# eovs/ldpc-lib

Hardware: AMD Instinct MI355X
Metric: decoded frames/sec, (2048,1024) QC-LDPC, 50 iters min-sum (higher is better)
Workload: dtype f64

## Files before the change

### include/ldpc_hip.h

```cpp
#ifndef LDPC_HIP_H
#define LDPC_HIP_H

#include <stdint.h>

#ifdef __cplusplus
extern "C" {
#endif

#define LDPC_HIP_ABI_VERSION 4

#define LDPC_HIP_BP_DEC 0
#define LDPC_HIP_SP_DEC 1
#define LDPC_HIP_ASP_DEC 2
#define LDPC_HIP_MS_DEC 3
#define LDPC_HIP_IMS_DEC 4
#define LDPC_HIP_IASP_DEC 5
#define LDPC_HIP_FHT_DEC 6
#define LDPC_HIP_TASP_DEC 7
#define LDPC_HIP_LMS_DEC 8
#define LDPC_HIP_LCHE_DEC 9

#define LDPC_HIP_EINVAL (-1)
#define LDPC_HIP_EUNSUPPORTED (-2)
#define LDPC_HIP_EHIP (-3)
// ... 4 lines not shown
int ldpc_hip_abi_version(void);
const char *ldpc_hip_last_error(void);
int ldpc_hip_device_count(void);

int ldpc_hip_open(int decoder_id, int rh, int nh, int M, const int16_t *hd, int device, ldpc_hip_ctx **out);
void ldpc_hip_close(ldpc_hip_ctx *ctx);

int ldpc_hip_n(const ldpc_hip_ctx *ctx);
int ldpc_hip_r(const ldpc_hip_ctx *ctx);
int ldpc_hip_edges(const ldpc_hip_ctx *ctx);
int ldpc_hip_hard_words(const ldpc_hip_ctx *ctx);
const char *ldpc_hip_kernel_name(const ldpc_hip_ctx *ctx);
int ldpc_hip_set_jit_mode(int mode);
int ldpc_hip_set_jit_mode_thread(int mode);
const char *ldpc_hip_last_launch(const ldpc_hip_ctx *ctx);

int ldpc_hip_decode_dev(ldpc_hip_ctx *ctx, const double *d_llr, long long B, int maxiter, double alpha,
                        uint32_t *d_hard, int32_t *d_iters, double *d_soft, void *stream);

int ldpc_hip_set_bp_chain(ldpc_hip_ctx *ctx, int on, int reset_carry);

int ldpc_hip_set_ims_params(ldpc_hip_ctx *ctx, double thr, int qbits, int dbits);

int ldpc_hip_decode_host(ldpc_hip_ctx *ctx, double *llr, long long B, int maxiter, int decision, double alpha,
                         double *decword, int32_t *iters, int clobber_sp_input);


int ldpc_hip_set_interleaver(ldpc_hip_ctx *ctx, int permutation_type, int permutation_block, int permutation_inter);
int ldpc_hip_set_codewords(ldpc_hip_ctx *ctx, const uint8_t *codewords, int ncw);

// ... 163 lines not shown
```

### ldpc-lib_amd/csrc/aot/ms_m64.hip

```cpp
#include "../ldpc_aot.hpp"

LDPC_AOT_KERNEL(ms_spec_appendix_c_m64_kernel, ms_m64_body, CodeAppendixCM64, 64, 2)
```

### ldpc-lib_amd/csrc/ldpc_aot.hpp

```cpp
#pragma once

#include <hip/hip_runtime.h>

#include "ldpc_spec.hpp"
#include "code_appendix_c_m64.hpp"

#define LDPC_AOT_DECLARE(name, threads, waves_per_simd) \
    __global__ void __launch_bounds__(threads, waves_per_simd) name(const ldpc_spec::SpecArgs a);
#define LDPC_AOT_KERNEL(name, body, Code, threads, waves_per_simd)                                   \
    __global__ void __launch_bounds__(threads, waves_per_simd) name(const ldpc_spec::SpecArgs a) {   \
        ldpc_spec::body<ldpc_spec::Code>(a);                                                         \
    }

LDPC_AOT_DECLARE(ms_spec_appendix_c_m64_kernel, 64, 2)
LDPC_AOT_DECLARE(ms_spec_appendix_c_m126_kernel, 128, 2)
LDPC_AOT_DECLARE(ms_chunk_appendix_c_m126_kernel, 64, 1)
LDPC_AOT_DECLARE(ms_spec_appendix_c_m512_kernel, 512, 2)
LDPC_AOT_DECLARE(ims_spec_appendix_c_m64_kernel, 64, 3)
LDPC_AOT_DECLARE(ims_spec_appendix_c_m126_kernel, 128, 2)
LDPC_AOT_DECLARE(lms_spec_appendix_c_m64_kernel, 64, 2)
LDPC_AOT_DECLARE(lms_spec_appendix_c_m512_kernel, 512, 2)
LDPC_AOT_DECLARE(sp_spec_appendix_c_m64_kernel, 512, 4)
LDPC_AOT_DECLARE(bp_spec_appendix_c_m64_kernel, 512, 4)
LDPC_AOT_DECLARE(asp_spec_appendix_c_m64_kernel, 512, 4)
LDPC_AOT_DECLARE(iasp_spec_appendix_c_m64_kernel, 512, 4)
LDPC_AOT_DECLARE(tasp_spec_appendix_c_m64_kernel, 128, 2)
LDPC_AOT_DECLARE(lche_spec_appendix_c_m64_kernel, 128, 2)
LDPC_AOT_DECLARE(tasp_spec_appendix_c_m126_kernel, 256, 2)
```

### ldpc-lib_amd/csrc/ldpc_hip.hip

```cpp
#include "../../include/ldpc_hip.h"
#include "../../include/ldpc/interleaver.h"
#include "../../include/ldpc/encoder.h"

#include <hip/hip_runtime.h>

#include <algorithm>
#include <cmath>
#include <cstdarg>
#include <cstdio>
#include <cstdlib>
#include <cstring>
#include <atomic>
#include <memory>
#include <string>
#include <type_traits>
#include <vector>

#include "ldpc_frontend.hpp"
#include "ldpc_jit.hpp"
#include "ldpc_kernels.hpp"
#include "ldpc_codeset.hpp"
#include "ldpc_codeset_wide.hpp"
#include "ldpc_codeset_sp.hpp"
#include "ldpc_global.hpp"
// ... 87 lines not shown
        for (int j = 0; same && j < rh; ++j) {
            same = (row_start[j + 1] - row_start[j]) == FC::RW[j];
            for (int e = row_start[j]; same && e < row_start[j + 1]; ++e)
                same = (int)(edges[e] >> 16) == FC::COL[j][e - row_start[j]] && (int)(edges[e] & 0xffffu) == FC::SH[j][e - row_start[j]];
        }
        return same;
    }
};

struct AotInstance {
    int decoder;
    const void *fn;
    int threads;
    const char *name;
    bool (CodeTables::*matches)() const;
};
const AotInstance kAot[] = {
    {LDPC_HIP_MS_DEC, (const void *)ms_spec_appendix_c_m64_kernel, 64, "ms_spec_appendix_c_m64_kernel", &CodeTables::is<ldpc_spec::CodeAppendixCM64>},
    {LDPC_HIP_MS_DEC, (const void *)ms_spec_appendix_c_m126_kernel, 128, "ms_spec_appendix_c_m126_kernel", &CodeTables::is<ldpc_spec::CodeAppendixCM126>},
    {LDPC_HIP_MS_DEC, (const void *)ms_chunk_appendix_c_m126_kernel, 64, "ms_chunk_appendix_c_m126_kernel", &CodeTables::is<ldpc_spec::CodeAppendixCM126>},
    {LDPC_HIP_MS_DEC, (const void *)ms_spec_appendix_c_m512_kernel, 512, "ms_spec_appendix_c_m512_kernel", &CodeTables::is<ldpc_spec::CodeAppendixCM512>},
    {LDPC_HIP_IMS_DEC, (const void *)ims_spec_appendix_c_m64_kernel, 64, "ims_spec_appendix_c_m64_kernel", &CodeTables::is<ldpc_spec::CodeAppendixCM64>},
    {LDPC_HIP_IMS_DEC, (const void *)ims_spec_appendix_c_m126_kernel, 128, "ims_spec_appendix_c_m126_kernel", &CodeTables::is<ldpc_spec::CodeAppendixCM126>},
    {LDPC_HIP_LMS_DEC, (const void *)lms_spec_appendix_c_m64_kernel, 64, "lms_spec_appendix_c_m64_kernel", &CodeTables::is<ldpc_spec::CodeAppendixCM64>},
    {LDPC_HIP_LMS_DEC, (const void *)lms_spec_appendix_c_m512_kernel, 512, "lms_spec_appendix_c_m512_kernel", &CodeTables::is<ldpc_spec::CodeAppendixCM512>},
    {LDPC_HIP_SP_DEC, (const void *)sp_spec_appendix_c_m64_kernel, 64 * ldpc_spec::kSpBodyWaves, "sp_spec_appendix_c_m64_kernel", &CodeTables::is<ldpc_spec::CodeAppendixCM64>},
    {LDPC_HIP_BP_DEC, (const void *)bp_spec_appendix_c_m64_kernel, 512, "bp_spec_appendix_c_m64_kernel", &CodeTables::is<ldpc_spec::CodeAppendixCM64>},
    {LDPC_HIP_ASP_DEC, (const void *)asp_spec_appendix_c_m64_kernel, 512, "asp_spec_appendix_c_m64_kernel", &CodeTables::is<ldpc_spec::CodeAppendixCM64>},
    {LDPC_HIP_IASP_DEC, (const void *)iasp_spec_appendix_c_m64_kernel, 512, "iasp_spec_appendix_c_m64_kernel", &CodeTables::is<ldpc_spec::CodeAppendixCM64>},
    {LDPC_HIP_LCHE_DEC, (const void *)lche_spec_appendix_c_m64_kernel, 128, "lche_spec_appendix_c_m64_kernel", &CodeTables::is<ldpc_spec::CodeAppendixCM64>},
    {LDPC_HIP_TASP_DEC, (const void *)tasp_spec_appendix_c_m64_kernel, 128, "tasp_spec_appendix_c_m64_kernel", &CodeTables::is<ldpc_spec::CodeAppendixCM64>},
    {LDPC_HIP_TASP_DEC, (const void *)tasp_spec_appendix_c_m126_kernel, 256, "tasp_spec_appendix_c_m126_kernel", &CodeTables::is<ldpc_spec::CodeAppendixCM126>},
};
// ... 73 lines not shown
    bool multiwave = false;
    bool have_generic = false;
    size_t lds_bytes = 0;
    double ims_thr = 1.4;
    int ims_qbits = 6, ims_dbits = 8;
    bool asp_cw2 = false;
    bool global_tier = false;
    char *d_glob_ws = nullptr;
    size_t glob_stride = 0;
    int glob_grid = 0;
    bool fast_m64 = false;
    int variant = 2;
    ldpc::FastTab fast_tab;
    const void *spec_aot = nullptr;
    const ldpc_jit::Kernel *spec_jit = nullptr;
    int spec_threads = 64;
    int spec_frames_per_block = 1;
    size_t spec_lds = 0;
    std::shared_ptr<ldpc_jit::Job> jit_job;
    std::string jit_name;
    bool global_is_fallback = false;
    unsigned *d_queue = nullptr;
    int persist_grid = 0;
    bool persist_jit = false;
    std::string kernel_name;
    std::string generic_name;
    const char *last_launch = "";
    bool bp_chain = true;
    std::vector<uint32_t> bp_carry;
    uint32_t *d_bp_stale = nullptr, *d_bp_synd = nullptr;
    int32_t *d_bp_idx = nullptr;
    long long bp_frames = 0;
    double *d_ims_coef = nullptr;
    long long ims_coef_frames = 0;
    int32_t *d_row_start = nullptr, *d_col_start = nullptr;
    uint32_t *d_edges = nullptr, *d_col_edges = nullptr, *d_col_slot = nullptr, *d_edge_row = nullptr;
    double *w_llr = nullptr;
    uint32_t *w_hard = nullptr;
    int32_t *w_iters = nullptr;
    double *w_soft = nullptr;
    unsigned long long *w_counters = nullptr;
    long long w_frames = 0;
// ... 95 lines not shown
        HIP_TRY(hipEventRecord(ev0, stream));
        return 0;
    }
    int end() {
        if (!c) return 0;
        HIP_TRY(hipEventRecord(ev1, stream));
        c->events.emplace_back(ev0, ev1);
        ev0 = ev1 = nullptr;
        return 0;
    }
    ~ProfTimer() { for (hipEvent_t e : {ev0, ev1}) if (e) (void)hipEventDestroy(e); }
};

struct SpecPlan { const char *body = nullptr; int threads = 0; size_t lds = 0; bool required = false; int frames_per_block = 1; };

constexpr size_t kLdsBudget = 160 * 1024 - 64;

int tasp_lane_regs(const CodeTables &t) {
    int regs = 85;
    for (int j = 0; j < t.rh; ++j) { const int L = (t.row_start[j + 1] - t.row_start[j] + 1) / 2; regs += 2 * L + (L + 1) / 2; }
    return regs;
}

SpecPlan plan_spec(int decoder_id, const CodeTables &t) {
    SpecPlan p;
    const int M = t.M, N = t.nh * t.M, W = (M + 63) / 64;
    const size_t soft_lds = sizeof(double) * (size_t)N + 16;
    if (!t.all_cols_used || t.max_rw > 16 || t.rh > 64 || t.nh > 64) return p;
    switch (decoder_id) {
    case LDPC_HIP_MS_DEC:
        if (M == 64) { p.body = "ms_m64_body"; p.threads = 64; p.lds = ldpc_spec::kMsM64LdsBytes((size_t)N); }
        else if (M <= 32) {
            p.body = "ms_small_body"; p.threads = 64; p.frames_per_block = 64 / M; p.lds = sizeof(double) * (size_t)N * (size_t)(64 / M);
        }
        else if (M > 64 && M <= 128 && !(getenv("LDPC_HIP_MS_CHUNK") && atoi(getenv("LDPC_HIP_MS_CHUNK")) == 0)) {
            p.body = "ms_chunk_body"; p.threads = 64; p.lds = sizeof(double) * (size_t)N;
        }
        else if (M >= 33 && M <= 512 && soft_lds <= kLdsBudget) { p.body = "ms_body"; p.threads = 64 * W; p.lds = soft_lds; }
        break;
    case LDPC_HIP_LMS_DEC:
        if (M <= 32) {
            p.body = "lms_small_body"; p.threads = 64; p.frames_per_block = 64 / M; p.lds = sizeof(double) * (size_t)N * (size_t)(64 / M);
        } else if (M >= 33 && M <= 512 && soft_lds <= kLdsBudget) { p.body = "lms_body"; p.threads = 64 * W; p.lds = soft_lds; }
        break;
    case LDPC_HIP_IMS_DEC: {
        const size_t lds = (((size_t)2 * N + 15) & ~(size_t)15) + (size_t)t.rh * 2 * LDPC_IMS_MSG_COPIES * M * 4 + 16;
// ... 140 lines not shown
        ga.d.ims_thr = c->ims_thr; ga.d.ims_qbits = c->ims_qbits; ga.d.ims_dbits = c->ims_dbits;
    }
    auto glaunch = [&](long long slots, const ChainIo &io) -> int {
        ga.slots = slots; ga.stale = io.stale; ga.synd_out = io.synd_out; ga.frame_idx = io.frame_idx;
        if (io.iters) ga.d.iters = io.iters;
        hipLaunchKernelGGL(kind.global, dim3((unsigned)(slots < grid ? slots : grid)), dim3((unsigned)ldpc::glob_threads(c->N)), 0, d.stream, ga);
        HIP_TRY(hipGetLastError());
        return 0;
    };
    if (c->decoder_id == LDPC_HIP_BP_DEC && c->bp_chain) return run_bp_chain(c, d.B, d.iters, d.stream, glaunch);
    ChainIo io;
    io.iters = d.iters;
    return glaunch(d.B, io);
}

int launch_spec(ldpc_hip_ctx *c, const decoder_kind &kind, const DecodeCall &d) {
    ldpc_spec::SpecArgs sa{};
    if (c->decoder_id == LDPC_HIP_IMS_DEC) {
        if (int rc = ims_scale(c, d.llr, d.B, d.stream)) return rc;
        sa.ims_coef = c->d_ims_coef; sa.ims_thr = c->ims_thr;
        sa.ims_max_quant = (1 << (c->ims_qbits - 1)) - 1; sa.ims_max_data = (1 << (c->ims_dbits - 1)) - 1; sa.ims_ialpha = ims_ialpha(d.alpha);
    }
    sa.llr = d.llr; sa.hard = d.hard; sa.iters = d.iters; sa.soft_out = d.soft; sa.maxiter = d.maxiter; sa.alpha = d.alpha;
    sa.nframes = d.B;
    static const bool persist_on = !(getenv("LDPC_HIP_PERSISTENT") && atoi(getenv("LDPC_HIP_PERSISTENT")) == 0);
    const bool persistent = persist_on && c->spec_frames_per_block == 1 && kind.queue;
    if (persistent) {
        if (!c->d_queue) HIP_TRY(hipMalloc(&c->d_queue, 64));
        if (c->persist_grid == 0 || c->persist_jit != (c->spec_aot == nullptr)) {
            int per_cu = 0, cus = 0;
            if (c->spec_aot) { if (int rc = set_lds_limit(c->spec_aot, c->spec_lds)) return rc; }
            hipError_t e = c->spec_aot ? hipOccupancyMaxActiveBlocksPerMultiprocessor(&per_cu, c->spec_aot, c->spec_threads, c->spec_lds)
                                       : hipModuleOccupancyMaxActiveBlocksPerMultiprocessor(&per_cu, c->spec_jit->fn, c->spec_threads, c->spec_lds);
            if (e != hipSuccess || per_cu < 1) { (void)hipGetLastError(); per_cu = 1; }
            HIP_TRY(hipDeviceGetAttribute(&cus, hipDeviceAttributeMultiprocessorCount, c->device));
            c->persist_grid = per_cu * (cus > 0 ? cus : 256);
            c->persist_jit = c->spec_aot == nullptr;
        }
    }
    auto launch = [&](long long frames) -> int {
        long long blocks = (frames + c->spec_frames_per_block - 1) / c->spec_frames_per_block;
        if (persistent && blocks > c->persist_grid) {
            HIP_TRY(hipMemsetAsync(c->d_queue, 0, sizeof(unsigned), d.stream));
            sa.queue = c->d_queue;
            blocks = c->persist_grid;
        }
        void *kargs[] = {&sa};
        if (c->spec_aot) {
            if (int rc = set_lds_limit(c->spec_aot, c->spec_lds)) return rc;
            HIP_TRY(hipLaunchKernel(c->spec_aot, dim3((unsigned)blocks), dim3((unsigned)c->spec_threads), kargs, c->spec_lds, d.stream));
        } else {
            HIP_TRY(hipModuleLaunchKernel(c->spec_jit->fn, (unsigned)blocks, 1, 1, (unsigned)c->spec_threads, 1, 1, (unsigned)c->spec_lds,
                                          d.stream, kargs, nullptr));
        }
        return 0;
    };
    if (c->decoder_id == LDPC_HIP_BP_DEC && c->bp_chain)
        return run_bp_chain(c, d.B, d.iters, d.stream, [&](long long frames, const ChainIo &io) -> int {
            sa.stale = io.stale; sa.synd_out = io.synd_out; sa.frame_idx = io.frame_idx; sa.iters = io.iters;
            return launch(frames);
        });
    return launch(d.B);
}

int launch_generic(ldpc_hip_ctx *c, const decoder_kind &kind, const DecodeCall &d) {
    ldpc::DecArgs a{};
    a.llr = d.llr; a.hard = d.hard; a.iters = d.iters; a.soft_out = d.soft;
// ... 87 lines not shown

    c->have_generic = have_generic;
    if (have_generic) c->generic_name = c->kernel_name;

    c->asp_cw2 = t.all_cw2;
    const bool can_global = !kind->global_min_rw2 || t.min_rw >= 2;
    const char *genv = getenv("LDPC_HIP_FORCE_GLOBAL");
    const bool forced_global = genv && atoi(genv) != 0;

    const SpecPlan plan = plan_spec(decoder_id, t);
    std::string why_not = plan.body ? "" : "this code shape has no code-specialised kernel";
    if (plan.body && (c->variant >= 2 || plan.required)) {
        c->spec_threads = plan.threads; c->spec_lds = plan.lds; c->spec_frames_per_block = plan.frames_per_block;
        for (const AotInstance &inst : kAot)
            if (inst.decoder == decoder_id && inst.threads == plan.threads && (t.*inst.matches)()) {
                c->spec_aot = inst.fn;
                c->kernel_name = std::string(inst.name) + " (ahead of time)";
                break;
            }
        const int jit_mode = jit_mode_effective();
        if (!c->spec_aot && jit_mode != 0 && !forced_global) {
            const bool has_fallback = have_generic || can_global;
            if (jit_mode == 2 && has_fallback) {
                c->spec_jit = ldpc_jit::get(device, plan.body, t.rows(), nh, M, why_not, false);
                if (!c->spec_jit) {
                    auto job = std::make_shared<ldpc_jit::Job>();
                    job->device = device; job->nh = nh; job->M = M; job->body = plan.body; job->rows = t.rows();
                    ldpc_jit::Worker::instance().submit(job);
                    c->jit_job = job;
                    c->jit_name = std::string(plan.body) + " instance (hiprtc)";
                    why_not = "its hiprtc instance is being compiled in the background";
                }
            } else {
                c->spec_jit = ldpc_jit::get(device, plan.body, t.rows(), nh, M, why_not);
            }
            if (c->spec_jit) c->kernel_name = std::string(plan.body) + " instance (hiprtc)";
        } else if (!c->spec_aot) {
            why_not = forced_global ? "LDPC_HIP_FORCE_GLOBAL" : "LDPC_HIP_JIT=0";
        }
    }
    if (can_global && (forced_global || (!c->spec_aot && !c->spec_jit && !have_generic))) {
        c->global_tier = true;
        c->global_is_fallback = c->jit_job != nullptr;
        c->spec_aot = nullptr; c->spec_jit = nullptr;
        c->kernel_name = kind->global_name;
    }
    if (c->global_tier || decoder_id == LDPC_HIP_IMS_DEC)
        c->glob_stride = ldpc::glob_ws_bytes(c->N, c->R, t.ne, M, kind->glob_edge_arrays);
    if (!c->spec_aot && !c->spec_jit && !c->global_tier) {
        if (!have_generic)
            return fail(LDPC_HIP_EUNSUPPORTED, "decoder %d, code %dx%d lifting %d: not supported by the generic kernel (limits: %d block rows, "
                        "%d block columns, row weight %d, M <= 512, 160 KiB LDS), no code-specialised instance: %s; the shape-unlimited "
                        "tier serves every built decoder; decoders 2, 5 and 7 need row weights >= 2, decoder 9 row weights <= 1024",
                        decoder_id, rh, nh, M, kRHM, kNHM, kRWM, why_not.c_str());
        if (plan.body && c->variant >= 2 && !c->jit_job)
// ... 9 lines not shown
    };
    HIP_TRY(upload(&c->d_row_start, t.row_start));
    HIP_TRY(upload(&c->d_col_start, t.col_start));
    HIP_TRY(upload(&c->d_edges, t.edges));
    HIP_TRY(upload(&c->d_col_edges, t.col_edges));
    HIP_TRY(upload(&c->d_col_slot, t.col_slot));
    HIP_TRY(upload(&c->d_edge_row, t.edge_row));
    HIP_TRY(hipMalloc(&c->w_counters, sizeof(unsigned long long) * 8));
    *out = c.release();
    return 0;
}

void ldpc_hip_close(ldpc_hip_ctx *c) {
    if (!c) return;
    if (c->jit_job) c->jit_job->cancelled.store(true);
    (void)hipSetDevice(c->device);
    free_workspace(c);
    if (c->d_row_start) (void)hipFree(c->d_row_start);
    if (c->d_col_start) (void)hipFree(c->d_col_start);
    if (c->d_edges) (void)hipFree(c->d_edges);
    if (c->d_col_edges) (void)hipFree(c->d_col_edges);
    if (c->d_col_slot) (void)hipFree(c->d_col_slot);
    if (c->d_edge_row) (void)hipFree(c->d_edge_row);
    if (c->w_counters) (void)hipFree(c->w_counters);
    if (c->d_queue) (void)hipFree(c->d_queue);
    if (c->d_ims_coef) (void)hipFree(c->d_ims_coef);
    if (c->d_bp_stale) (void)hipFree(c->d_bp_stale);
    if (c->d_bp_synd) (void)hipFree(c->d_bp_synd);
    if (c->d_bp_idx) (void)hipFree(c->d_bp_idx);
    if (c->d_glob_ws) (void)hipFree(c->d_glob_ws);
// ... 19 lines not shown
    adopt_jit(const_cast<ldpc_hip_ctx *>(c));
    return c->kernel_name.c_str();
}

int ldpc_hip_set_jit_mode(int mode) {
    if (mode < 0 || mode > 2) return fail(LDPC_HIP_EINVAL, "ldpc_hip_set_jit_mode: 0 (never), 1 (inside ldpc_hip_open) or 2 (in the background)");
    return g_jit_mode.exchange(mode);
}
int ldpc_hip_set_jit_mode_thread(int mode) {
    if (mode < -1 || mode > 2) return fail(LDPC_HIP_EINVAL, "ldpc_hip_set_jit_mode_thread: -1 (no override), 0, 1 or 2");
    const int before = t_jit_mode;
    t_jit_mode = mode;
    return before;
}
const char *ldpc_hip_last_launch(const ldpc_hip_ctx *c) { return c ? c->last_launch : ""; }

int ldpc_hip_decode_dev(ldpc_hip_ctx *c, const double *d_llr, long long B, int maxiter, double alpha,
                        uint32_t *d_hard, int32_t *d_iters, double *d_soft, void *stream_) {
    if (!c || B < 0) return fail(LDPC_HIP_EINVAL, "ldpc_hip_decode_dev: bad argument");
    if (B == 0) return 0;
    if (!d_llr) return fail(LDPC_HIP_EINVAL, "ldpc_hip_decode_dev: null llr");
    if (B > 0x7fffffffLL) return fail(LDPC_HIP_EINVAL, "batch too large");
    if (maxiter < 1) return fail(LDPC_HIP_EINVAL, "ldpc_hip_decode_dev: maxiter must be >= 1 (got %d)", maxiter);
    if (int rc = set_device(c)) return rc;
    hipStream_t stream = (hipStream_t)stream_;
    adopt_jit(c);

    ProfTimer timer;
    if (int rc = timer.begin(c, stream)) return rc;
    const decoder_kind &kind = *decoder_find(c->decoder_id);
    const DecodeCall d{d_llr, B, maxiter, alpha, d_hard, d_iters, d_soft, stream};
    bool use_spec = c->spec_aot || c->spec_jit;
    bool use_global = c->global_tier;
    const int ialpha = ims_ialpha(alpha);
    if (use_spec && c->decoder_id == LDPC_HIP_IMS_DEC && (c->ims_dbits > 8 || c->ims_qbits > 8 || ialpha < 0 || ialpha > 16)) {
        use_spec = false;
        if (!c->have_generic) use_global = true;
    }
    c->last_launch = use_global ? kind.global_name : use_spec ? c->kernel_name.c_str() : c->generic_name.c_str();
    if (int rc = use_global ? launch_global(c, kind, d) : use_spec ? launch_spec(c, kind, d) : launch_generic(c, kind, d)) return rc;
    HIP_TRY(hipGetLastError());
    return timer.end();
}

int ldpc_hip_decode_host(ldpc_hip_ctx *c, double *llr, long long B, int maxiter, int decision, double alpha,
                         double *decword, int32_t *iters, int clobber_sp_input) {
    if (!c || !llr || B < 0) return fail(LDPC_HIP_EINVAL, "ldpc_hip_decode_host: bad argument");
    if (B == 0) return 0;
    if (int rc = set_device(c)) return rc;
    const decoder_kind &kind = *decoder_find(c->decoder_id);
    const bool sp = kind.soft_is_input;
    if (kind.ignores_decision) decision = 0;
    const bool need_soft = decision != 0 || (sp && clobber_sp_input);
    if (int rc = ensure_workspace(c, B, need_soft)) return rc;
// ... 448 lines not shown
```

### ldpc-lib_amd/csrc/ldpc_jit.hpp

```cpp
#pragma once

#include <dlfcn.h>
#include <sys/stat.h>
#include <unistd.h>
#include <hip/hip_runtime.h>

#include <atomic>
#include <condition_variable>
#include <cstdio>
#include <cstdlib>
#include <deque>
#include <fstream>
#include <iterator>
#include <map>
#include <memory>
#include <mutex>
#include <sstream>
#include <string>
#include <thread>
#include <vector>

namespace ldpc_jit {

struct Kernel {
// ... 65 lines not shown
      << "    static constexpr int SH[" << rh << "][" << wmax << "] = {" << sh.str() << "};\n"
      << "    static constexpr int FIRST[" << rh << "][" << wmax << "] = {" << fi.str() << "};\n"
      << "};\n";
    return o.str();
}

inline std::string this_library_dir() {
    Dl_info info;
    if (!dladdr(reinterpret_cast<void *>(&this_library_dir), &info) || !info.dli_fname) return ".";
    std::string p = info.dli_fname;
    const size_t k = p.find_last_of('/');
    return k == std::string::npos ? "." : p.substr(0, k);
}

inline const Kernel *get(int device, const char *body, const std::vector<std::vector<std::pair<int, int>>> &rows, int nh,
                         int M, std::string &err, bool compile = true) {
    static std::mutex mu;
    static std::map<std::string, Kernel> &cache = *new std::map<std::string, Kernel>();
    const std::string code = code_struct(rows, nh, M);
    const bool eight_waves = std::string(body) == "sp_body" || std::string(body) == "asp_body" || std::string(body) == "iasp_body" ||
                             std::string(body) == "bp_body";
    const bool tasp = std::string(body) == "tasp_body" || std::string(body) == "lche_body";
    int tasp_regs = 85;
    for (const auto &r : rows) tasp_regs += 2 * (((int)r.size() + 1) / 2) + (((int)r.size() + 1) / 2 + 1) / 2;
    const int threads = eight_waves ? 512 : std::string(body) == "ms_chunk_body" ? 64 : tasp ? ((2 * M + 63) / 64) * 64 : ((M + 63) / 64) * 64;
    const std::string key = std::to_string(device) + "|" + body + "|" + code;
    auto lookup = [&]() -> const Kernel * {
        std::lock_guard<std::mutex> lk(mu);
        auto it = cache.find(key);
        return it != cache.end() ? &it->second : nullptr;
    };
// ... 13 lines not shown
    const std::string hdr = hs.str();
    const std::string tab_path = this_library_dir() + "/csrc/lche_table.hpp";
    std::ifstream tf(tab_path);
    if (!tf) { err = "cannot read " + tab_path; return nullptr; }
    std::stringstream ts;
    ts << tf.rdbuf();
    const std::string tab = ts.str();
    const std::string src = "#include \"ldpc_spec.hpp\"\nnamespace {\n" + code +
                            "}\nextern \"C\" __global__ void __launch_bounds__(" + std::to_string(threads) + (eight_waves ? ", 4" : ((tasp && tasp_regs > 256) || std::string(body) == "ms_chunk_body") ? ", 1" : ", 2") + ") spec_jit(const ldpc_spec::SpecArgs a) {\n"
                            "    ldpc_spec::" + body + "<Code>(a);\n}\n";
    std::string cache_file;
    std::string cache_dir;
    if (const char *dir = getenv("LDPC_HIP_CACHE_DIR")) cache_dir = dir;
    else if (const char *x = getenv("XDG_CACHE_HOME")) cache_dir = std::string(x) + "/ldpc_hip";
    else if (const char *h = getenv("HOME")) cache_dir = std::string(h) + "/.cache/ldpc_hip";
    if (cache_dir == "off" || cache_dir == "0") cache_dir.clear();
    if (!cache_dir.empty()) {
        for (size_t i = 1; i <= cache_dir.size(); ++i)
            if (i == cache_dir.size() || cache_dir[i] == '/') (void)mkdir(cache_dir.substr(0, i).c_str(), 0755);
        const char *dir = cache_dir.c_str();
        unsigned long long h = 1469598103934665603ull;
        auto mix = [&](const std::string &t) { for (unsigned char ch : t) { h ^= ch; h *= 1099511628211ull; } };
        mix(src); mix(hdr); mix(tab); mix("gfx950 -O3 -ffp-contract=off");
        int rt_version = 0;
        (void)hipRuntimeGetVersion(&rt_version);
        mix("rt" + std::to_string(rt_version));
        hipDeviceProp_t prop;
        if (hipGetDeviceProperties(&prop, device) == hipSuccess) mix(prop.gcnArchName);
        char name[64];
        snprintf(name, sizeof name, "/ldpc_spec_%016llx.hsaco", h);
        cache_file = std::string(dir) + name;
// ... 38 lines not shown
    }
    if (!cache_file.empty()) {
        static std::atomic<unsigned> tmp_serial{0};
        const std::string tmp = cache_file + ".tmp" + std::to_string((long long)getpid()) + "." + std::to_string(tmp_serial.fetch_add(1));
        std::ofstream of(tmp, std::ios::binary);
        if (of && of.write(bin.data(), (std::streamsize)bin.size()) && (of.close(), true)) {
            if (rename(tmp.c_str(), cache_file.c_str()) != 0) (void)remove(tmp.c_str());
        }
    }
    return publish(k);
}

struct Job {
    int device = 0, nh = 0, M = 0;
    std::string body;
    std::vector<std::vector<std::pair<int, int>>> rows;
    std::atomic<int> state{0};
    std::atomic<bool> cancelled{false};
    const Kernel *kernel = nullptr;
    std::string err;
};

class Worker {
public:
    static Worker &instance() {
        static Worker *w = new Worker();
        return *w;
    }
    void submit(const std::shared_ptr<Job> &j) {
        std::lock_guard<std::mutex> lk(mu_);
// ... 25 lines not shown
        const char *opts[] = {"--offload-arch=gfx950", "-O1"};
        (void)r->CompileProgram(prog, 2, opts);
        r->DestroyProgram(&prog);
    }
    void run() {
        for (;;) {
            std::shared_ptr<Job> j;
            {
                std::unique_lock<std::mutex> lk(mu_);
                cv_.wait(lk, [this] { return stop_ || !q_.empty(); });
                if (stop_) return;
                j = q_.back();
                q_.pop_back();
            }
            if (j->cancelled.load()) { j->state.store(2); continue; }
            j->kernel = get(j->device, j->body.c_str(), j->rows, j->nh, j->M, j->err, true);
            j->state.store(j->kernel ? 1 : 2, std::memory_order_release);
        }
    }
    std::mutex mu_;
    std::condition_variable cv_;
    std::deque<std::shared_ptr<Job>> q_;
    std::thread th_;
    bool started_ = false, stop_ = false;
};

}
```

### ldpc-lib_amd/csrc/ldpc_spec.hpp

```cpp
#pragma once

#ifndef __HIPCC_RTC__
#include <hip/hip_runtime.h>
#endif
#include "lche_table.hpp"

namespace ldpc_spec {

typedef unsigned int u32;
typedef unsigned long long u64;

struct SpecArgs {
    const double *llr;
    u32 *hard;
    int *iters;
    double *soft_out;
    int maxiter;
    double alpha;
    const u32 *stale;
    u32 *synd_out;
    const int *frame_idx;
    const double *ims_coef;
    double ims_thr;
    int ims_max_quant, ims_max_data, ims_ialpha;
// ... 364 lines not shown
template <int KPCAP>
constexpr int ms_m64_prefix_rows(int kr) { return KPCAP < kr ? (KPCAP > 0 ? KPCAP : 0) : kr; }

template <class C>
constexpr int ms_m64_nonlocal_cols() {
    int n = 0;
    for (int k = 0; k < C::NH; ++k) n += ms_m64_local_col<C>(k) ? 0 : 1;
    return n;
}
template <class C>
constexpr int ms_m64_nonlocal_col(int n) {
    for (int k = 0; k < C::NH; ++k)
        if (!ms_m64_local_col<C>(k) && n-- == 0) return k;
    return -1;
}
constexpr int kMsM64YDepth = 8;
template <class C>
constexpr int ms_m64_y_in_flight_r23() {
    int peak = 0;
    for (int k0 = 0; k0 < C::NH; k0 += 8) {
        int n = 0;
        for (int k = k0; k < C::NH && k < k0 + 24; ++k) n += ms_m64_local_col<C>(k) ? 0 : 1;
        peak = n > peak ? n : peak;
    }
    return peak;
}
constexpr int kMsM64State3Regs = 244;
template <class C>
constexpr int ms_m64_state3_regs(int rows) {
    int e = 0;
    for (int j = 0; j < rows; ++j) e += C::RW[j];
    return 2 * e + 5 * (C::RH - rows) + 4 * C::WMAX - 2;
}
template <class C, int YD>
constexpr int ms_m64_carry_rows() {
    constexpr int nl = ms_m64_nonlocal_cols<C>(), depth = YD < nl ? YD : nl, was = ms_m64_y_in_flight_r23<C>();
    constexpr int base = ms_m64_keep_rows<C>(ms_m64_keep_budget<C>());
    constexpr int more = base > 0 ? ms_m64_keep_rows<C>(ms_m64_keep_budget<C>() + 2 * (was > depth ? was - depth : 0)) : 0;
    int rows = base;
    while (rows < more && ms_m64_state3_regs<C>(rows + 1) <= kMsM64State3Regs) ++rows;
    return rows;
}

template <class C, int KPCAP = 1 << 30, int YD = kMsM64YDepth, int YROW = -1, int KRSET = -1>
__device__ __forceinline__ void ms_m64_body(const SpecArgs &a) {
    static_assert(C::M == 64, "ms_m64_body: one frame per wavefront needs M == 64");
    static_assert(YD >= 1 && YROW >= -1 && YROW < C::RH && KRSET <= C::RH, "ms_m64_body: switch out of range");
    constexpr int RH = C::RH, NH = C::NH, N = C::NH * 64;
    constexpr int KR = KRSET >= 0 ? KRSET : ms_m64_carry_rows<C, YD>();
    typedef IC<ms_m64_prefix_rows<KPCAP>(KR)> KP;
    extern __shared__ double lds[];
    const int lane = threadIdx.x;
    const double alpha = a.alpha, alpha_mag = fabs(a.alpha);
    long long fr = blockIdx.x;

    const u32 lane8 = (u32)lane * 8u;
    const u32 lo = lds_addr(lds) + lane8, hi = lo + 512u;
    auto at = [&](u32 tie, auto S, auto K) -> double * {
        constexpr int c = decltype(S)::value, k = decltype(K)::value;
        static_assert(c >= 0 && c < 64 && k * 512 + c * 8 < 65536, "shift / block column out of range");
        if constexpr (c == 0) return lds_at(hi + (u32)(k * 512));
        else return lds_at(sel32_tied(hi, lo, ~0ull << (64 - c), tie) + (u32)(k * 512 + c * 8));
    };
    auto own = [&](auto K) -> double * { return lds_at(hi + (u32)(decltype(K)::value * 512)); };

  while (fr < a.nframes) {
    const __amdgpu_buffer_rsrc_t ybuf = __builtin_amdgcn_make_buffer_rsrc(const_cast<double *>(a.llr + fr * N), 0, N * 8, 0x00020000);

    double m1[RH], m2[RH];
    u32 meta[RH];
    double keep[RH][C::WMAX];
    static_for<0, RH>([&](auto J) {
        constexpr int j = decltype(J)::value;
        m1[j] = 0.0; m2[j] = 0.0; meta[j] = 0u;
        if constexpr (j < KR) static_for<0, C::RW[j]>([&](auto S) { keep[j][decltype(S)::value] = 0.0; });
    });

    int res = -a.maxiter;
    for (int iter = 0; iter < a.maxiter; ++iter) {
        constexpr int NL = ms_m64_nonlocal_cols<C>(), YAHEAD = YD < NL ? YD : NL;
        double y[NH];
        auto load_y = [&](auto N0, auto N1) {
            if constexpr (decltype(N0)::value < NL && decltype(N0)::value < decltype(N1)::value) {
u32 so = 0;
                asm volatile("" : "+s"(so));
                static_for<decltype(N0)::value, (decltype(N1)::value < NL ? decltype(N1)::value : NL)>([&](auto I) {
                    constexpr int k = ms_m64_nonlocal_col<C>(decltype(I)::value);
                    typedef u32 u32x2 __attribute__((ext_vector_type(2)));
                    const u32x2 v = __builtin_amdgcn_raw_buffer_load_b64(ybuf, (int)lane8, (int)(so + (u32)(k * 512)), 0);
                    y[k] = mk(v.y, v.x);
                });
            }
        };
        double yl[NH], soft_l[NH];
        auto load_yl = [&](auto JN) {
            constexpr int jn = decltype(JN)::value;
            if constexpr (ms_m64_local_starts<C>(jn) > 0) {
                u32 so = 0;
                asm volatile("" : "+s"(so));
                static_for<0, C::RW[jn]>([&](auto S) {
                    constexpr int k = C::COL[jn][decltype(S)::value];
                    if constexpr (ms_m64_local_col<C>(k) && ms_m64_first_row<C>(k) == jn) {
// ... 34 lines not shown
                        double *p = at(mt, IC<C::SH[j][s]>{}, IC<C::COL[j][s]>{});
                        if constexpr (C::FIRST[j][s]) *p = cv;
                        else __hip_atomic_fetch_add(p, cv, __ATOMIC_RELAXED, __HIP_MEMORY_SCOPE_WORKGROUP);
                    }
                });
            }
            __builtin_amdgcn_sched_barrier(0);
            if constexpr (j == YROW) {
                load_y(IC<0>{}, IC<YAHEAD>{});
                __builtin_amdgcn_sched_barrier(0);
            }
        });
        if constexpr (YROW < 0) load_y(IC<0>{}, IC<YAHEAD>{});
        static_for<0, NL>([&](auto I) {
            constexpr int i = decltype(I)::value, k = ms_m64_nonlocal_col<C>(i);
            if constexpr (i % 2 == 0) load_y(IC<i + YAHEAD>{}, IC<i + YAHEAD + 2>{});
            double *p = own(IC<k>{});
            const double pr = *p * alpha;
            *p = (y[k] + 0.0) + pr;
            if constexpr (i % 2 == 1) __builtin_amdgcn_sched_barrier(0);
        });
        load_yl(IC<0>{});
        u32 failw = 0;
        static_for<0, RH>([&](auto J) {
            constexpr int j = decltype(J)::value;
            constexpr int RW = C::RW[j];
            u32 mt = meta[j];
            asm volatile("" : "+v"(mt));
            load_yl(IC<j + 1>{});
            double nm1 = kMaxVal, nm2 = kMaxVal;
            u32 npos = 0, nS = 0, sy = 0;
            double r[RW], tt_[RW];
            static_for<0, RW>([&](auto S) {
                constexpr int s = decltype(S)::value;
                constexpr int k = C::COL[j][s];
// ... 5 lines not shown
                        static_for<j, ms_m64_last_row<C>(k) + 1>([&](auto JJ) {
                            constexpr int jj = decltype(JJ)::value, ss = ms_m64_slot_of<C>(jj, k);
                            if constexpr (ss >= 0) {
                                if constexpr (jj >= KR) {
                                    const u32 m = jj == j ? mt : meta[jj];
                                    const double aa = sel64(m1[jj], m2[jj], lanes_eq(m & 0xffu, (u32)ss));
                                    keep[jj][ss] = signed_mag(aa, ss == 0 ? m : ss == 1 ? twice(m) : m << ss);
                                }
                                const double cv = keep[jj][ss];
                                if constexpr (jj == j) acc = cv;
                                else acc = acc + cv;
                            }
                        });
                        const double pr = acc * alpha;
                        soft_l[k] = (yl[k] + 0.0) + pr;
                        *own(IC<k>{}) = soft_l[k];
                    }
                    r[s] = soft_l[k];
                }
            });
            auto step = [&](auto S, double x) {
                constexpr int s = decltype(S)::value;
                const double tt = r[s] - x;
                nS = __builtin_amdgcn_alignbit(nS, hi32(tt), 31);
                const double v = fabs(tt);
                if constexpr (j < KR) tt_[s] = tt;
                if constexpr (s == 0) {
                    nm1 = fmin(v, kMaxVal);
                } else if constexpr (j < KR) {
                    nm2 = fmin(fmax(v, nm1), nm2);
                    nm1 = fmin(v, nm1);
// ... 64 lines not shown
                        W = twice(W);
                    });
                }
            } else {
                m1[j] = nm1; m2[j] = nm2; meta[j] = ((nS ^ (0u - (__popc(nS) & 1u))) << (32 - RW)) | npos;
            }
            __builtin_amdgcn_sched_barrier(0);
        });
        if (__ballot((failw >> 31) != 0) == 0ull) { res = iter + 1; break; }
    }

    int ol = lane;
    if constexpr (KR > 0) asm volatile("" : "+v"(ol));
    if (lane == 0 && a.iters) a.iters[fr] = res;
    if (a.hard) {
        u64 mine = 0ull;
        static_for<0, NH>([&](auto K) {
            constexpr int k = decltype(K)::value;
            const u64 b = __ballot((hi32(*own(K)) >> 31) != 0);
            if (ol == k) mine = b;
        });
        if (ol < NH) reinterpret_cast<u64 *>(a.hard + fr * (N / 32))[ol] = mine;
    }
    if (a.soft_out) {
        static_for<0, NH>([&](auto K) {
            constexpr int k = decltype(K)::value;
            a.soft_out[fr * N + k * 64 + ol] = *own(K);
        });
    }
    if (!a.queue) break;
    u32 ticket = 0;
    if (lane == 0) ticket = atomicAdd(a.queue, 1u);
    fr = (long long)gridDim.x + (long long)(u32)__builtin_amdgcn_readfirstlane((int)ticket);
  }
}

template <class C>
__device__ __forceinline__ void ms_body(const SpecArgs &a) {
    constexpr int RH = C::RH, NH = C::NH, M = C::M, N = NH * M, W = (M + 63) / 64;
    constexpr bool POW2 = (M & (M - 1)) == 0;
    extern __shared__ double lds[];
    char *const ldsb = reinterpret_cast<char *>(lds);
    int *const flag = reinterpret_cast<int *>(ldsb + (size_t)N * 8);
    const int n = threadIdx.x;
    const bool valid = (M % 64 == 0) || n < M;
    const u32 n8 = (u32)(valid ? n : 0) * 8u;
    const double alpha = a.alpha;
    for_each_frame<true>(a, (long long)blockIdx.x, [&](const long long fr) {

    auto rot = [&](u32 base, auto S) -> u32 {
// ... 1818 lines not shown
```

Before: 6.413 million.

## Cache channel LLRs in spare LDS and add hard-only MS M64 kernel variant

Each frame now gets a larger LDS share, and the spare slots hold the channel LLRs of non-local columns. This avoids reloading them from global memory on every iteration. A hard-decision-only variant (SOFT=false) drops the LDS stores of local soft values and keeps their signs in register bitmasks, which frees the local-column LDS slots for more resident LLRs. The host picks this variant when no soft output is requested, with separate persistent-grid sizing per variant. The larger per-frame LDS share may lower occupancy, and the extra bitmask registers add register pressure.

```diff
diff --git a/include/ldpc_hip.h b/include/ldpc_hip.h
--- a/include/ldpc_hip.h
+++ b/include/ldpc_hip.h
@@ -42,6 +42,7 @@
 int ldpc_hip_set_jit_mode(int mode);
 int ldpc_hip_set_jit_mode_thread(int mode);
 const char *ldpc_hip_last_launch(const ldpc_hip_ctx *ctx);
+int ldpc_hip_last_launch_without_soft(const ldpc_hip_ctx *ctx);
 
 int ldpc_hip_decode_dev(ldpc_hip_ctx *ctx, const double *d_llr, long long B, int maxiter, double alpha,
                         uint32_t *d_hard, int32_t *d_iters, double *d_soft, void *stream);
diff --git a/ldpc-lib_amd/csrc/aot/ms_m64.hip b/ldpc-lib_amd/csrc/aot/ms_m64.hip
--- a/ldpc-lib_amd/csrc/aot/ms_m64.hip
+++ b/ldpc-lib_amd/csrc/aot/ms_m64.hip
@@ -1,3 +1,4 @@
 #include "../ldpc_aot.hpp"
 
 LDPC_AOT_KERNEL(ms_spec_appendix_c_m64_kernel, ms_m64_body, CodeAppendixCM64, 64, 2)
+LDPC_AOT_KERNEL(ms_spec_appendix_c_m64_hard_kernel, ms_m64_hard_body, CodeAppendixCM64, 64, 2)
diff --git a/ldpc-lib_amd/csrc/ldpc_aot.hpp b/ldpc-lib_amd/csrc/ldpc_aot.hpp
--- a/ldpc-lib_amd/csrc/ldpc_aot.hpp
+++ b/ldpc-lib_amd/csrc/ldpc_aot.hpp
@@ -13,6 +13,7 @@
     }
 
 LDPC_AOT_DECLARE(ms_spec_appendix_c_m64_kernel, 64, 2)
+LDPC_AOT_DECLARE(ms_spec_appendix_c_m64_hard_kernel, 64, 2)
 LDPC_AOT_DECLARE(ms_spec_appendix_c_m126_kernel, 128, 2)
 LDPC_AOT_DECLARE(ms_chunk_appendix_c_m126_kernel, 64, 1)
 LDPC_AOT_DECLARE(ms_spec_appendix_c_m512_kernel, 512, 2)
diff --git a/ldpc-lib_amd/csrc/ldpc_hip.hip b/ldpc-lib_amd/csrc/ldpc_hip.hip
--- a/ldpc-lib_amd/csrc/ldpc_hip.hip
+++ b/ldpc-lib_amd/csrc/ldpc_hip.hip
@@ -125,9 +125,11 @@
     int threads;
     const char *name;
     bool (CodeTables::*matches)() const;
+    const void *fn_hard = nullptr;
 };
 const AotInstance kAot[] = {
-    {LDPC_HIP_MS_DEC, (const void *)ms_spec_appendix_c_m64_kernel, 64, "ms_spec_appendix_c_m64_kernel", &CodeTables::is<ldpc_spec::CodeAppendixCM64>},
+    {LDPC_HIP_MS_DEC, (const void *)ms_spec_appendix_c_m64_kernel, 64, "ms_spec_appendix_c_m64_kernel", &CodeTables::is<ldpc_spec::CodeAppendixCM64>,
+     (const void *)ms_spec_appendix_c_m64_hard_kernel},
     {LDPC_HIP_MS_DEC, (const void *)ms_spec_appendix_c_m126_kernel, 128, "ms_spec_appendix_c_m126_kernel", &CodeTables::is<ldpc_spec::CodeAppendixCM126>},
     {LDPC_HIP_MS_DEC, (const void *)ms_chunk_appendix_c_m126_kernel, 64, "ms_chunk_appendix_c_m126_kernel", &CodeTables::is<ldpc_spec::CodeAppendixCM126>},
     {LDPC_HIP_MS_DEC, (const void *)ms_spec_appendix_c_m512_kernel, 512, "ms_spec_appendix_c_m512_kernel", &CodeTables::is<ldpc_spec::CodeAppendixCM512>},
@@ -231,6 +233,11 @@
     ldpc::FastTab fast_tab;
     const void *spec_aot = nullptr;
     const ldpc_jit::Kernel *spec_jit = nullptr;
+    bool spec_has_hard = false;
+    const void *spec_aot_hard = nullptr;
+    const ldpc_jit::Kernel *spec_jit_hard = nullptr;
+    std::shared_ptr<ldpc_jit::Job> jit_job_hard;
+    std::vector<std::vector<std::pair<int, int>>> spec_rows;
     int spec_threads = 64;
     int spec_frames_per_block = 1;
     size_t spec_lds = 0;
@@ -238,11 +245,12 @@
     std::string jit_name;
     bool global_is_fallback = false;
     unsigned *d_queue = nullptr;
-    int persist_grid = 0;
-    bool persist_jit = false;
+    const void *persist_for[2] = {nullptr, nullptr};
+    int persist_grid[2] = {0, 0};
     std::string kernel_name;
     std::string generic_name;
     const char *last_launch = "";
+    bool last_without_soft = false;
     bool bp_chain = true;
     std::vector<uint32_t> bp_carry;
     uint32_t *d_bp_stale = nullptr, *d_bp_synd = nullptr;
@@ -368,7 +376,7 @@
 
 struct SpecPlan { const char *body = nullptr; int threads = 0; size_t lds = 0; bool required = false; int frames_per_block = 1; };
 
-constexpr size_t kLdsBudget = 160 * 1024 - 64;
+constexpr size_t kLdsBudget = ldpc_spec::kMsM64LdsBudget;
 
 int tasp_lane_regs(const CodeTables &t) {
     int regs = 85;
@@ -383,7 +391,7 @@
     if (!t.all_cols_used || t.max_rw > 16 || t.rh > 64 || t.nh > 64) return p;
     switch (decoder_id) {
     case LDPC_HIP_MS_DEC:
-        if (M == 64) { p.body = "ms_m64_body"; p.threads = 64; p.lds = ldpc_spec::kMsM64LdsBytes((size_t)N); }
+        if (M == 64) { p.body = "ms_m64_body"; p.threads = 64; p.lds = ldpc_spec::kMsM64FrameLdsBytes((size_t)N); }
         else if (M <= 32) {
             p.body = "ms_small_body"; p.threads = 64; p.frames_per_block = 64 / M; p.lds = sizeof(double) * (size_t)N * (size_t)(64 / M);
         }
@@ -554,6 +562,29 @@
     return glaunch(d.B, io);
 }
 
+int jit_hard_instance(ldpc_hip_ctx *c) {
+    if (c->spec_jit_hard) return 0;
+    std::string err;
+    if (c->jit_job_hard) {
+        const int st = c->jit_job_hard->state.load(std::memory_order_acquire);
+        if (st == 0) return 0;
+        const ldpc_jit::Kernel *k = c->jit_job_hard->kernel;
+        err = c->jit_job_hard->err;
+        c->jit_job_hard.reset();
+        if (st == 1) { c->spec_jit_hard = k; return 0; }
+        return fail(LDPC_HIP_EUNSUPPORTED, "ms_m64_hard_body: no hiprtc instance (%s)", err.c_str());
+    }
+    const bool background = jit_mode_effective() == 2;
+    c->spec_jit_hard = ldpc_jit::get(c->device, "ms_m64_hard_body", c->spec_rows, c->nh, c->M, err, !background, false);
+    if (c->spec_jit_hard) return 0;
+    if (!background) return fail(LDPC_HIP_EUNSUPPORTED, "ms_m64_hard_body: no hiprtc instance (%s)", err.c_str());
+    auto job = std::make_shared<ldpc_jit::Job>();
+    job->device = c->device; job->nh = c->nh; job->M = c->M; job->body = "ms_m64_hard_body"; job->disk = false; job->rows = c->spec_rows;
+    ldpc_jit::Worker::instance().submit(job);
+    c->jit_job_hard = job;
+    return 0;
+}
+
 int launch_spec(ldpc_hip_ctx *c, const decoder_kind &kind, const DecodeCall &d) {
     ldpc_spec::SpecArgs sa{};
     if (c->decoder_id == LDPC_HIP_IMS_DEC) {
@@ -565,32 +596,43 @@
     sa.nframes = d.B;
     static const bool persist_on = !(getenv("LDPC_HIP_PERSISTENT") && atoi(getenv("LDPC_HIP_PERSISTENT")) == 0);
     const bool persistent = persist_on && c->spec_frames_per_block == 1 && kind.queue;
+    const void *aot = c->spec_aot;
+    const ldpc_jit::Kernel *jit = c->spec_jit;
+    int which = 0;
+    if (c->spec_has_hard && !d.soft) {
+        if (c->spec_aot) aot = c->spec_aot_hard;
+        else if (int rc = jit_hard_instance(c)) return rc;
+        else if (c->spec_jit_hard) jit = c->spec_jit_hard;
+        which = (aot != c->spec_aot || jit != c->spec_jit) ? 1 : 0;
+    }
+    c->last_without_soft = which == 1;
     if (persistent) {
         if (!c->d_queue) HIP_TRY(hipMalloc(&c->d_queue, 64));
-        if (c->persist_grid == 0 || c->persist_jit != (c->spec_aot == nullptr)) {
+        const void *key = aot ? aot : (const void *)jit->fn;
+        if (c->persist_for[which] != key) {
             int per_cu = 0, cus = 0;
-            if (c->spec_aot) { if (int rc = set_lds_limit(c->spec_aot, c->spec_lds)) return rc; }
-            hipError_t e = c->spec_aot ? hipOccupancyMaxActiveBlocksPerMultiprocessor(&per_cu, c->spec_aot, c->spec_threads, c->spec_lds)
-                                       : hipModuleOccupancyMaxActiveBlocksPerMultiprocessor(&per_cu, c->spec_jit->fn, c->spec_threads, c->spec_lds);
+            if (aot) { if (int rc = set_lds_limit(aot, c->spec_lds)) return rc; }
+            hipError_t e = aot ? hipOccupancyMaxActiveBlocksPerMultiprocessor(&per_cu, aot, c->spec_threads, c->spec_lds)
+                               : hipModuleOccupancyMaxActiveBlocksPerMultiprocessor(&per_cu, jit->fn, c->spec_threads, c->spec_lds);
             if (e != hipSuccess || per_cu < 1) { (void)hipGetLastError(); per_cu = 1; }
             HIP_TRY(hipDeviceGetAttribute(&cus, hipDeviceAttributeMultiprocessorCount, c->device));
-            c->persist_grid = per_cu * (cus > 0 ? cus : 256);
-            c->persist_jit = c->spec_aot == nullptr;
+            c->persist_grid[which] = per_cu * (cus > 0 ? cus : 256);
+            c->persist_for[which] = key;
         }
     }
     auto launch = [&](long long frames) -> int {
         long long blocks = (frames + c->spec_frames_per_block - 1) / c->spec_frames_per_block;
-        if (persistent && blocks > c->persist_grid) {
+        if (persistent && blocks > c->persist_grid[which]) {
             HIP_TRY(hipMemsetAsync(c->d_queue, 0, sizeof(unsigned), d.stream));
             sa.queue = c->d_queue;
-            blocks = c->persist_grid;
+            blocks = c->persist_grid[which];
         }
         void *kargs[] = {&sa};
-        if (c->spec_aot) {
-            if (int rc = set_lds_limit(c->spec_aot, c->spec_lds)) return rc;
-            HIP_TRY(hipLaunchKernel(c->spec_aot, dim3((unsigned)blocks), dim3((unsigned)c->spec_threads), kargs, c->spec_lds, d.stream));
+        if (aot) {
+            if (int rc = set_lds_limit(aot, c->spec_lds)) return rc;
+            HIP_TRY(hipLaunchKernel(aot, dim3((unsigned)blocks), dim3((unsigned)c->spec_threads), kargs, c->spec_lds, d.stream));
         } else {
-            HIP_TRY(hipModuleLaunchKernel(c->spec_jit->fn, (unsigned)blocks, 1, 1, (unsigned)c->spec_threads, 1, 1, (unsigned)c->spec_lds,
+            HIP_TRY(hipModuleLaunchKernel(jit->fn, (unsigned)blocks, 1, 1, (unsigned)c->spec_threads, 1, 1, (unsigned)c->spec_lds,
                                           d.stream, kargs, nullptr));
         }
         return 0;
@@ -708,7 +750,7 @@
         c->spec_threads = plan.threads; c->spec_lds = plan.lds; c->spec_frames_per_block = plan.frames_per_block;
         for (const AotInstance &inst : kAot)
             if (inst.decoder == decoder_id && inst.threads == plan.threads && (t.*inst.matches)()) {
-                c->spec_aot = inst.fn;
+                c->spec_aot = inst.fn; c->spec_aot_hard = inst.fn_hard;
                 c->kernel_name = std::string(inst.name) + " (ahead of time)";
                 break;
             }
@@ -733,6 +775,10 @@
             why_not = forced_global ? "LDPC_HIP_FORCE_GLOBAL" : "LDPC_HIP_JIT=0";
         }
     }
+    if (plan.body && std::string(plan.body) == "ms_m64_body") {
+        c->spec_has_hard = c->spec_aot ? c->spec_aot_hard != nullptr : true;
+        if (!c->spec_aot) c->spec_rows = t.rows();
+    }
     if (can_global && (forced_global || (!c->spec_aot && !c->spec_jit && !have_generic))) {
         c->global_tier = true;
         c->global_is_fallback = c->jit_job != nullptr;
@@ -772,6 +818,7 @@
 void ldpc_hip_close(ldpc_hip_ctx *c) {
     if (!c) return;
     if (c->jit_job) c->jit_job->cancelled.store(true);
+    if (c->jit_job_hard) c->jit_job_hard->cancelled.store(true);
     (void)hipSetDevice(c->device);
     free_workspace(c);
     if (c->d_row_start) (void)hipFree(c->d_row_start);
@@ -821,6 +868,7 @@
     return before;
 }
 const char *ldpc_hip_last_launch(const ldpc_hip_ctx *c) { return c ? c->last_launch : ""; }
+int ldpc_hip_last_launch_without_soft(const ldpc_hip_ctx *c) { return c && c->last_without_soft ? 1 : 0; }
 
 int ldpc_hip_decode_dev(ldpc_hip_ctx *c, const double *d_llr, long long B, int maxiter, double alpha,
                         uint32_t *d_hard, int32_t *d_iters, double *d_soft, void *stream_) {
@@ -845,6 +893,7 @@
         if (!c->have_generic) use_global = true;
     }
     c->last_launch = use_global ? kind.global_name : use_spec ? c->kernel_name.c_str() : c->generic_name.c_str();
+    c->last_without_soft = false;
     if (int rc = use_global ? launch_global(c, kind, d) : use_spec ? launch_spec(c, kind, d) : launch_generic(c, kind, d)) return rc;
     HIP_TRY(hipGetLastError());
     return timer.end();
diff --git a/ldpc-lib_amd/csrc/ldpc_jit.hpp b/ldpc-lib_amd/csrc/ldpc_jit.hpp
--- a/ldpc-lib_amd/csrc/ldpc_jit.hpp
+++ b/ldpc-lib_amd/csrc/ldpc_jit.hpp
@@ -103,7 +103,7 @@
 }
 
 inline const Kernel *get(int device, const char *body, const std::vector<std::vector<std::pair<int, int>>> &rows, int nh,
-                         int M, std::string &err, bool compile = true) {
+                         int M, std::string &err, bool compile = true, bool disk = true) {
     static std::mutex mu;
     static std::map<std::string, Kernel> &cache = *new std::map<std::string, Kernel>();
     const std::string code = code_struct(rows, nh, M);
@@ -147,7 +147,7 @@
     if (const char *dir = getenv("LDPC_HIP_CACHE_DIR")) cache_dir = dir;
     else if (const char *x = getenv("XDG_CACHE_HOME")) cache_dir = std::string(x) + "/ldpc_hip";
     else if (const char *h = getenv("HOME")) cache_dir = std::string(h) + "/.cache/ldpc_hip";
-    if (cache_dir == "off" || cache_dir == "0") cache_dir.clear();
+    if (cache_dir == "off" || cache_dir == "0" || !disk) cache_dir.clear();
     if (!cache_dir.empty()) {
         for (size_t i = 1; i <= cache_dir.size(); ++i)
             if (i == cache_dir.size() || cache_dir[i] == '/') (void)mkdir(cache_dir.substr(0, i).c_str(), 0755);
@@ -216,6 +216,7 @@
 struct Job {
     int device = 0, nh = 0, M = 0;
     std::string body;
+    bool disk = true;
     std::vector<std::vector<std::pair<int, int>>> rows;
     std::atomic<int> state{0};
     std::atomic<bool> cancelled{false};
@@ -271,7 +272,7 @@
                 q_.pop_back();
             }
             if (j->cancelled.load()) { j->state.store(2); continue; }
-            j->kernel = get(j->device, j->body.c_str(), j->rows, j->nh, j->M, j->err, true);
+            j->kernel = get(j->device, j->body.c_str(), j->rows, j->nh, j->M, j->err, true, j->disk);
             j->state.store(j->kernel ? 1 : 2, std::memory_order_release);
         }
     }
diff --git a/ldpc-lib_amd/csrc/ldpc_spec.hpp b/ldpc-lib_amd/csrc/ldpc_spec.hpp
--- a/ldpc-lib_amd/csrc/ldpc_spec.hpp
+++ b/ldpc-lib_amd/csrc/ldpc_spec.hpp
@@ -402,6 +402,50 @@
         if (!ms_m64_local_col<C>(k) && n-- == 0) return k;
     return -1;
 }
+constexpr unsigned long kMsM64LdsBudget = 160 * 1024 - 64;
+constexpr int kMsM64FramesPerCu = 8;
+constexpr unsigned long kMsM64FrameLdsBytes(unsigned long n) {
+    const unsigned long fit = kMsM64LdsBudget / kMsM64LdsBytes(n), frames = fit < kMsM64FramesPerCu ? fit : kMsM64FramesPerCu;
+    const unsigned long share = frames ? kMsM64LdsBudget / frames / 512 * 512 : 0;
+    return share > kMsM64LdsBytes(n) ? share : kMsM64LdsBytes(n);
+}
+template <class C>
+constexpr int ms_m64_spare_cols() { return (int)((kMsM64FrameLdsBytes(C::NH * 64) - kMsM64LdsBytes(C::NH * 64)) / 512); }
+template <class C>
+constexpr int ms_m64_local_cols() { return C::NH - ms_m64_nonlocal_cols<C>(); }
+template <class C, bool SOFT>
+constexpr int ms_m64_resident_cols() {
+    const int room = ms_m64_spare_cols<C>() + (SOFT ? 0 : ms_m64_local_cols<C>()), nl = ms_m64_nonlocal_cols<C>();
+    return room < nl ? room : nl;
+}
+template <class C>
+constexpr int ms_m64_resident_slot(int i) {
+    const int spare = ms_m64_spare_cols<C>();
+    if (i < spare) return C::NH + i;
+    int n = i - spare;
+    for (int k = 0; k < C::NH; ++k)
+        if (ms_m64_local_col<C>(k) && n-- == 0) return k;
+    return -1;
+}
+template <class C>
+constexpr int ms_m64_local_place(int k) {
+    int p = 0;
+    for (int j = 0; j < C::RH; ++j)
+        for (int s = 0; s < C::RW[j]; ++s) {
+            const int kk = C::COL[j][s];
+            if (ms_m64_local_col<C>(kk) && ms_m64_first_row<C>(kk) == j) {
+                if (kk == k) return p;
+                ++p;
+            }
+        }
+    return -1;
+}
+template <class C>
+constexpr int ms_m64_local_bit(int k) {
+    const int p = ms_m64_local_place<C>(k), w = p / 32, left = ms_m64_local_cols<C>() - 32 * w;
+    return (left < 32 ? left : 32) - 1 - (p - 32 * w);
+}
+
 constexpr int kMsM64YDepth = 8;
 template <class C>
 constexpr int ms_m64_y_in_flight_r23() {
@@ -430,11 +474,15 @@
     return rows;
 }
 
-template <class C, int KPCAP = 1 << 30, int YD = kMsM64YDepth, int YROW = -1, int KRSET = -1>
+template <class C, int KPCAP = 1 << 30, int YD = kMsM64YDepth, int YROW = -1, int KRSET = -1, bool SOFT = true, int RSET = -1, int BITW = -1>
 __device__ __forceinline__ void ms_m64_body(const SpecArgs &a) {
     static_assert(C::M == 64, "ms_m64_body: one frame per wavefront needs M == 64");
     static_assert(YD >= 1 && YROW >= -1 && YROW < C::RH && KRSET <= C::RH, "ms_m64_body: switch out of range");
+    static_assert(RSET <= ms_m64_resident_cols<C, SOFT>() && (SOFT || BITW != 0), "ms_m64_body: switch out of range");
     constexpr int RH = C::RH, NH = C::NH, N = C::NH * 64;
+    constexpr int RES = RSET >= 0 ? RSET : ms_m64_resident_cols<C, SOFT>();
+    constexpr bool BITS = BITW < 0 ? !SOFT : BITW != 0;
+    constexpr int NLOC = ms_m64_local_cols<C>(), HBW = BITS ? (NLOC + 31) / 32 : 0;
     constexpr int KR = KRSET >= 0 ? KRSET : ms_m64_carry_rows<C, YD>();
     typedef IC<ms_m64_prefix_rows<KPCAP>(KR)> KP;
     extern __shared__ double lds[];
@@ -454,6 +502,12 @@
 
   while (fr < a.nframes) {
     const __amdgpu_buffer_rsrc_t ybuf = __builtin_amdgcn_make_buffer_rsrc(const_cast<double *>(a.llr + fr * N), 0, N * 8, 0x00020000);
+    static_for<0, RES>([&](auto I) {
+        constexpr int i = decltype(I)::value, k = ms_m64_nonlocal_col<C>(i);
+        typedef u32 u32x2 __attribute__((ext_vector_type(2)));
+        const u32x2 v = __builtin_amdgcn_raw_buffer_load_b64(ybuf, (int)lane8, k * 512, 0);
+        *own(IC<ms_m64_resident_slot<C>(i)>{}) = mk(v.y, v.x) + 0.0;
+    });
 
     double m1[RH], m2[RH];
     u32 meta[RH];
@@ -464,16 +518,18 @@
         if constexpr (j < KR) static_for<0, C::RW[j]>([&](auto S) { keep[j][decltype(S)::value] = 0.0; });
     });
 
+    u32 hb[HBW > 0 ? HBW : 1];
+    static_for<0, HBW>([&](auto W) { hb[decltype(W)::value] = 0u; });
     int res = -a.maxiter;
     for (int iter = 0; iter < a.maxiter; ++iter) {
-        constexpr int NL = ms_m64_nonlocal_cols<C>(), YAHEAD = YD < NL ? YD : NL;
+        constexpr int NL = ms_m64_nonlocal_cols<C>(), NS = NL - RES, YAHEAD = YD < NS ? YD : NS;
         double y[NH];
         auto load_y = [&](auto N0, auto N1) {
-            if constexpr (decltype(N0)::value < NL && decltype(N0)::value < decltype(N1)::value) {
-u32 so = 0;
+            if constexpr (decltype(N0)::value < NS && decltype(N0)::value < decltype(N1)::value) {
+                u32 so = 0;
                 asm volatile("" : "+s"(so));
-                static_for<decltype(N0)::value, (decltype(N1)::value < NL ? decltype(N1)::value : NL)>([&](auto I) {
-                    constexpr int k = ms_m64_nonlocal_col<C>(decltype(I)::value);
+                static_for<decltype(N0)::value, (decltype(N1)::value < NS ? decltype(N1)::value : NS)>([&](auto I) {
+                    constexpr int k = ms_m64_nonlocal_col<C>(RES + decltype(I)::value);
                     typedef u32 u32x2 __attribute__((ext_vector_type(2)));
                     const u32x2 v = __builtin_amdgcn_raw_buffer_load_b64(ybuf, (int)lane8, (int)(so + (u32)(k * 512)), 0);
                     y[k] = mk(v.y, v.x);
@@ -538,11 +594,17 @@
         if constexpr (YROW < 0) load_y(IC<0>{}, IC<YAHEAD>{});
         static_for<0, NL>([&](auto I) {
             constexpr int i = decltype(I)::value, k = ms_m64_nonlocal_col<C>(i);
-            if constexpr (i % 2 == 0) load_y(IC<i + YAHEAD>{}, IC<i + YAHEAD + 2>{});
             double *p = own(IC<k>{});
-            const double pr = *p * alpha;
-            *p = (y[k] + 0.0) + pr;
-            if constexpr (i % 2 == 1) __builtin_amdgcn_sched_barrier(0);
+            if constexpr (i < RES) {
+                const double yc = *own(IC<ms_m64_resident_slot<C>(i)>{});
+                const double pr = *p * alpha;
+                *p = yc + pr;
+            } else {
+                if constexpr ((i - RES) % 2 == 0) load_y(IC<i - RES + YAHEAD>{}, IC<i - RES + YAHEAD + 2>{});
+                const double pr = *p * alpha;
+                *p = (y[k] + 0.0) + pr;
+            }
+            if constexpr (i < RES ? i % 2 == 1 : (i - RES) % 2 == 1) __builtin_amdgcn_sched_barrier(0);
         });
         load_yl(IC<0>{});
         u32 failw = 0;
@@ -578,7 +640,11 @@
                         });
                         const double pr = acc * alpha;
                         soft_l[k] = (yl[k] + 0.0) + pr;
-                        *own(IC<k>{}) = soft_l[k];
+                        if constexpr (BITS) {
+                            constexpr int w = ms_m64_local_place<C>(k) / 32;
+                            hb[w] = __builtin_amdgcn_alignbit(hb[w], hi32(soft_l[k]), 31);
+                        }
+                        if constexpr (SOFT) *own(IC<k>{}) = soft_l[k];
                     }
                     r[s] = soft_l[k];
                 }
@@ -673,19 +739,34 @@
     if constexpr (KR > 0) asm volatile("" : "+v"(ol));
     if (lane == 0 && a.iters) a.iters[fr] = res;
     if (a.hard) {
+        auto sign_of = [&] {
+            if constexpr (BITS) {
+                u32 ho[HBW > 0 ? HBW : 1];
+                static_for<0, HBW>([&](auto W) { ho[decltype(W)::value] = hb[decltype(W)::value]; asm volatile("" : "+v"(ho[decltype(W)::value])); });
+                return [&, ho](auto K) -> u32 {
+                    constexpr int k = decltype(K)::value;
+                    if constexpr (ms_m64_local_col<C>(k)) {
+                        constexpr int w = ms_m64_local_place<C>(k) / 32, up = 31 - ms_m64_local_bit<C>(k);
+                        return ho[w] << up >> 31;
+                    } else return hi32(*own(K)) >> 31;
+                };
+            } else return [&](auto K) -> u32 { return hi32(*own(K)) >> 31; };
+        }();
         u64 mine = 0ull;
         static_for<0, NH>([&](auto K) {
             constexpr int k = decltype(K)::value;
-            const u64 b = __ballot((hi32(*own(K)) >> 31) != 0);
+            const u64 b = __ballot(sign_of(K) != 0);
             if (ol == k) mine = b;
         });
         if (ol < NH) reinterpret_cast<u64 *>(a.hard + fr * (N / 32))[ol] = mine;
     }
-    if (a.soft_out) {
-        static_for<0, NH>([&](auto K) {
-            constexpr int k = decltype(K)::value;
-            a.soft_out[fr * N + k * 64 + ol] = *own(K);
-        });
+    if constexpr (SOFT) {
+        if (a.soft_out) {
+            static_for<0, NH>([&](auto K) {
+                constexpr int k = decltype(K)::value;
+                a.soft_out[fr * N + k * 64 + ol] = *own(K);
+            });
+        }
     }
     if (!a.queue) break;
     u32 ticket = 0;
@@ -693,6 +774,8 @@
     fr = (long long)gridDim.x + (long long)(u32)__builtin_amdgcn_readfirstlane((int)ticket);
   }
 }
+template <class C>
+__device__ __forceinline__ void ms_m64_hard_body(const SpecArgs &a) { ms_m64_body<C, 1 << 30, kMsM64YDepth, -1, -1, false>(a); }
 
 template <class C>
 __device__ __forceinline__ void ms_body(const SpecArgs &a) {
```

After: 6.876 million, median of 6. 1.07x the previous value.
